# jiwoon-ahn/irn

Measured on NVIDIA H100. Metric: pseudo-label images/sec (CAM+random-walk), higher is better.
Workload: dtype f32

## Files before the change

### irn_b200/csrc/conv_wgmma.cuh

```cuda
#pragma once
#include <cuda.h>
#include <cuda_runtime.h>
#include <cstdint>
#include <type_traits>

#include "tma.cuh"

namespace irn {

constexpr int kTcTW = 16, kTcTH = 8;
constexpr int kTcBK = 32;
constexpr int kBfBK = 64;
constexpr int kWgThreads = 384;

struct TcMaps {
    CUtensorMap a;
    CUtensorMap b_hi;
    CUtensorMap b_lo;
    CUtensorMap a2;
};

struct TcArgs {
    const float* bias;
    const float* residual;
// ... 72 lines not shown
          "+f"(d[24]), "+f"(d[25]), "+f"(d[26]), "+f"(d[27]), "+f"(d[28]), "+f"(d[29]), "+f"(d[30]), "+f"(d[31]),
          "+f"(d[32]), "+f"(d[33]), "+f"(d[34]), "+f"(d[35]), "+f"(d[36]), "+f"(d[37]), "+f"(d[38]), "+f"(d[39]),
          "+f"(d[40]), "+f"(d[41]), "+f"(d[42]), "+f"(d[43]), "+f"(d[44]), "+f"(d[45]), "+f"(d[46]), "+f"(d[47]),
          "+f"(d[48]), "+f"(d[49]), "+f"(d[50]), "+f"(d[51]), "+f"(d[52]), "+f"(d[53]), "+f"(d[54]), "+f"(d[55]),
          "+f"(d[56]), "+f"(d[57]), "+f"(d[58]), "+f"(d[59]), "+f"(d[60]), "+f"(d[61]), "+f"(d[62]), "+f"(d[63])
        : "r"(a[0]), "r"(a[1]), "r"(a[2]), "r"(a[3]), "l"(db), "r"(scale_d));
}

template <> __device__ __forceinline__ void wg_mma<true, 64>(float (&d)[32], const uint32_t (&a)[4], uint64_t db, uint32_t scale_d) {
    asm volatile(
        "{\n\t.reg .pred p;\n\tsetp.ne.b32 p, %37, 0;\n\t"
        "wgmma.mma_async.sync.aligned.m64n64k16.f32.f16.f16 {"
        "%0, %1, %2, %3, %4, %5, %6, %7, %8, %9, %10, %11, %12, %13, %14, %15, "
        "%16, %17, %18, %19, %20, %21, %22, %23, %24, %25, %26, %27, %28, %29, %30, %31"
        "}, {%32, %33, %34, %35}, %36, p, 1, 1, 0;\n\t}"
        : "+f"(d[0]), "+f"(d[1]), "+f"(d[2]), "+f"(d[3]), "+f"(d[4]), "+f"(d[5]), "+f"(d[6]), "+f"(d[7]),
          "+f"(d[8]), "+f"(d[9]), "+f"(d[10]), "+f"(d[11]), "+f"(d[12]), "+f"(d[13]), "+f"(d[14]), "+f"(d[15]),
          "+f"(d[16]), "+f"(d[17]), "+f"(d[18]), "+f"(d[19]), "+f"(d[20]), "+f"(d[21]), "+f"(d[22]), "+f"(d[23]),
          "+f"(d[24]), "+f"(d[25]), "+f"(d[26]), "+f"(d[27]), "+f"(d[28]), "+f"(d[29]), "+f"(d[30]), "+f"(d[31])
        : "r"(a[0]), "r"(a[1]), "r"(a[2]), "r"(a[3]), "l"(db), "r"(scale_d));
}

template <> __device__ __forceinline__ void wg_mma<true, 128>(float (&d)[64], const uint32_t (&a)[4], uint64_t db, uint32_t scale_d) {
    asm volatile(
        "{\n\t.reg .pred p;\n\tsetp.ne.b32 p, %69, 0;\n\t"
        "wgmma.mma_async.sync.aligned.m64n128k16.f32.f16.f16 {"
        "%0, %1, %2, %3, %4, %5, %6, %7, %8, %9, %10, %11, %12, %13, %14, %15, "
        "%16, %17, %18, %19, %20, %21, %22, %23, %24, %25, %26, %27, %28, %29, %30, %31, "
        "%32, %33, %34, %35, %36, %37, %38, %39, %40, %41, %42, %43, %44, %45, %46, %47, "
        "%48, %49, %50, %51, %52, %53, %54, %55, %56, %57, %58, %59, %60, %61, %62, %63"
        "}, {%64, %65, %66, %67}, %68, p, 1, 1, 0;\n\t}"
        : "+f"(d[0]), "+f"(d[1]), "+f"(d[2]), "+f"(d[3]), "+f"(d[4]), "+f"(d[5]), "+f"(d[6]), "+f"(d[7]),
          "+f"(d[8]), "+f"(d[9]), "+f"(d[10]), "+f"(d[11]), "+f"(d[12]), "+f"(d[13]), "+f"(d[14]), "+f"(d[15]),
          "+f"(d[16]), "+f"(d[17]), "+f"(d[18]), "+f"(d[19]), "+f"(d[20]), "+f"(d[21]), "+f"(d[22]), "+f"(d[23]),
          "+f"(d[24]), "+f"(d[25]), "+f"(d[26]), "+f"(d[27]), "+f"(d[28]), "+f"(d[29]), "+f"(d[30]), "+f"(d[31]),
          "+f"(d[32]), "+f"(d[33]), "+f"(d[34]), "+f"(d[35]), "+f"(d[36]), "+f"(d[37]), "+f"(d[38]), "+f"(d[39]),
          "+f"(d[40]), "+f"(d[41]), "+f"(d[42]), "+f"(d[43]), "+f"(d[44]), "+f"(d[45]), "+f"(d[46]), "+f"(d[47]),
          "+f"(d[48]), "+f"(d[49]), "+f"(d[50]), "+f"(d[51]), "+f"(d[52]), "+f"(d[53]), "+f"(d[54]), "+f"(d[55]),
          "+f"(d[56]), "+f"(d[57]), "+f"(d[58]), "+f"(d[59]), "+f"(d[60]), "+f"(d[61]), "+f"(d[62]), "+f"(d[63])
        : "r"(a[0]), "r"(a[1]), "r"(a[2]), "r"(a[3]), "l"(db), "r"(scale_d));
}

__device__ __forceinline__ float tf32_hi(float x) { return __uint_as_float((__float_as_uint(x) + 0x1000u) & 0xFFFFE000u); }

__device__ __forceinline__ void f16_split2(float a, float b, uint32_t& hi, uint32_t& lo) {
    asm("cvt.rz.satfinite.f16x2.f32 %0, %1, %2;" : "=r"(hi) : "f"(b), "f"(a));
    const float ha = __uint_as_float(__float_as_uint(a) & 0xFFFFE000u), hb = __uint_as_float(__float_as_uint(b) & 0xFFFFE000u);
    asm("cvt.rn.satfinite.f16x2.f32 %0, %1, %2;" : "=r"(lo) : "f"(b - hb), "f"(a - ha));
}

template <bool F16>
__device__ __forceinline__ void wg_load_frag(const unsigned char* row, int k, int key, int t4, float (&v)[8]) {
    if (F16) {
        const unsigned char* box = row + (k >> 1) * 16384;
        const int c = 4 * (k & 1) + (t4 >> 1);
        const float2 x0 = *reinterpret_cast<const float2*>(box + ((c ^ key) << 4));
        const float2 x1 = *reinterpret_cast<const float2*>(box + 1024 + ((c ^ key) << 4));
        const float2 x2 = *reinterpret_cast<const float2*>(box + (((c + 2) ^ key) << 4));
        const float2 x3 = *reinterpret_cast<const float2*>(box + 1024 + (((c + 2) ^ key) << 4));
        v[0] = x0.x; v[1] = x0.y; v[2] = x1.x; v[3] = x1.y; v[4] = x2.x; v[5] = x2.y; v[6] = x3.x; v[7] = x3.y;
    } else {
        const int c = 2 * k;
        v[0] = *reinterpret_cast<const float*>(row + ((c ^ key) << 4));
        v[1] = *reinterpret_cast<const float*>(row + 1024 + ((c ^ key) << 4));
        v[2] = *reinterpret_cast<const float*>(row + (((c + 1) ^ key) << 4));
        v[3] = *reinterpret_cast<const float*>(row + 1024 + (((c + 1) ^ key) << 4));
    }
}

template <bool F16>
__device__ __forceinline__ void wg_split_frag(const float (&v)[8], uint32_t (&hi)[4], uint32_t (&lo)[4]) {
#pragma unroll
    for (int i = 0; i < 4; ++i) {
        if (F16) {
            f16_split2(v[2 * i], v[2 * i + 1], hi[i], lo[i]);
        } else {
            const float h = tf32_hi(v[i]);
            hi[i] = __float_as_uint(h);
            lo[i] = __float_as_uint(v[i] - h);
        }
    }
}

template <bool F16, int BN>
__global__ void __launch_bounds__(kWgThreads, 1)
conv_wg_kernel(const __grid_constant__ TcMaps maps, const TcArgs args) {
    using Cfg = WgCfg<F16, BN>;
    constexpr int S = Cfg::kStages;
    constexpr int R = BN / 2;
    extern __shared__ unsigned char wg_smem_raw[];
    unsigned char* smem = wg_smem_raw + ((1024u - (smem_u32(wg_smem_raw) & 1023u)) & 1023u);
    uint64_t* bars = (uint64_t*)(smem + S * Cfg::kStageBytes);
    uint64_t* full = bars;
    uint64_t* empty = bars + S;

    const int warp = threadIdx.x >> 5, lane = threadIdx.x & 31;
    const int n_tiles = args.Cout / BN;
    const int n_items = args.tiles_x * args.tiles_y * args.B * n_tiles;
    const int cblocks = args.Cin / Cfg::kBK;
    const int KB = (!F16 && args.stem) ? args.ksize : args.ksize * args.ksize * cblocks;

    if (threadIdx.x == 0) {
        for (int s = 0; s < S; ++s) {
            mbar_init(&full[s], 1);
            mbar_init(&empty[s], 8);
        }
        fence_mbar_init();
    }
    __syncthreads();

    if (warp < 4) {
        setmaxnreg_dec<kWgProducerRegs>();
        if (threadIdx.x == 0) {
            tma_prefetch_desc(&maps.a);
            tma_prefetch_desc(&maps.b_hi);
            tma_prefetch_desc(&maps.b_lo);
            if (F16 && args.kb_split < KB) tma_prefetch_desc(&maps.a2);
            int s = 0;
            uint32_t ph = 0;
            for (int item = blockIdx.x; item < n_items; item += gridDim.x) {
                const int tile = item / n_tiles;
                const int ox0 = (tile % args.tiles_x) * kTcTW;
                const int oy0 = ((tile / args.tiles_x) % args.tiles_y) * kTcTH;
                const int b = tile / (args.tiles_x * args.tiles_y);
                const int n0 = (item % n_tiles) * BN;
                for (int kb = 0; kb < KB; ++kb) {
                    mbar_wait(&empty[s], ph ^ 1);
                    unsigned char* st = smem + s * Cfg::kStageBytes;
                    unsigned char* wb = st + Cfg::kARaw;
                    mbar_arrive_expect_tx(&full[s], (uint32_t)Cfg::kStageBytes);
                    if (args.stem) {
                        const int row = F16 ? 2 * kb : kb;
                        tma_load_4d(st, &maps.a, &full[s], 0, ox0, oy0 * 2 + row, b);
                        if (F16) tma_load_4d(st + 16384, &maps.a, &full[s], 0, ox0, oy0 * 2 + row + 1, b);
                    } else {
                        const bool second = F16 && kb >= args.kb_split;
                        const CUtensorMap* am = second ? &maps.a2 : &maps.a;
                        const int tap = second ? 0 : kb / cblocks, cb = second ? kb - args.kb_split : kb % cblocks;
                        const int r = tap / args.ksize, ss = tap % args.ksize;
                        const int x = second ? ox0 * args.stride2 : ox0 * args.stride - args.pad + ss;
                        const int y = second ? oy0 * args.stride2 : oy0 * args.stride - args.pad + r;
                        tma_load_4d(st, am, &full[s], cb * Cfg::kBK, x, y, b);
                        if (F16) tma_load_4d(st + 16384, am, &full[s], cb * Cfg::kBK + 32, x, y, b);
                    }
                    tma_load_2d(wb, &maps.b_hi, &full[s], kb * Cfg::kBK, n0);
                    tma_load_2d(wb + Cfg::kBBytes, &maps.b_lo, &full[s], kb * Cfg::kBK, n0);
                    if (++s == S) { s = 0; ph ^= 1; }
                }
            }
        }
        return;
    }

    setmaxnreg_inc<kWgConsumerRegs>();
    const int g = (threadIdx.x >> 7) - 1, wq = warp & 3;
    const int key = lane >> 2, t4 = lane & 3;
    const int frag_off = (64 * g + 16 * wq + key) * 128 + (F16 ? 8 * (t4 & 1) : 4 * t4);
    float acc[R], part[2][R];
    uint32_t fa[2][2][4];
    int s = 0, s_prev = 0;
    uint32_t ph = 0;
    auto promote = [&](auto P) {
        constexpr int p = decltype(P)::value;
        wg_fence_regs(part[p]);
#pragma unroll
        for (int i = 0; i < R; ++i) acc[i] += part[p][i];
        __syncwarp();
        if (lane == 0) mbar_arrive(&empty[s_prev]);
    };
    auto kblock = [&](auto P) {
        constexpr int p = decltype(P)::value;
        mbar_wait(&full[s], ph);
        unsigned char* st = smem + s * Cfg::kStageBytes;
        const unsigned char* frag = st + frag_off;
        const uint32_t b_hi = smem_u32(st + Cfg::kARaw), b_lo = b_hi + Cfg::kBBytes;
#pragma unroll
        for (int k = 0; k < 4; ++k) {
            float v[8];
            wg_load_frag<F16>(frag, k, key, t4, v);
            wg_wait<1>();
            if (p == 1 && k == 1) promote(std::integral_constant<int, 0>());
            wg_split_frag<F16>(v, fa[k & 1][0], fa[k & 1][1]);
            if (k == 0) wg_fence_regs(part[p]);
            wg_fence();
            const uint64_t db_hi = wg_desc(b_hi + 32 * k), db_lo = wg_desc(b_lo + 32 * k);
            wg_mma<F16, BN>(part[p], fa[k & 1][0], db_hi, k != 0 ? 1u : 0u);
            wg_mma<F16, BN>(part[p], fa[k & 1][1], db_hi, 1u);
            wg_mma<F16, BN>(part[p], fa[k & 1][0], db_lo, 1u);
            wg_commit();
        }
        s_prev = s;
        if (++s == S) { s = 0; ph ^= 1; }
    };

    for (int item = blockIdx.x; item < n_items; item += gridDim.x) {
        const int tile = item / n_tiles;
        const int ox0 = (tile % args.tiles_x) * kTcTW;
        const int oy0 = ((tile / args.tiles_x) % args.tiles_y) * kTcTH;
        const int b = tile / (args.tiles_x * args.tiles_y);
        const int n0 = (item % n_tiles) * BN;
#pragma unroll
        for (int i = 0; i < R; ++i) acc[i] = 0.f;
        int kb = 0;
        for (; kb + 1 < KB; kb += 2) {
            kblock(std::integral_constant<int, 0>());
            kblock(std::integral_constant<int, 1>());
            wg_wait<0>();
            promote(std::integral_constant<int, 1>());
        }
        if (kb < KB) {
            kblock(std::integral_constant<int, 0>());
            wg_wait<0>();
            promote(std::integral_constant<int, 0>());
        }

#pragma unroll
        for (int h = 0; h < 2; ++h) {
            const int row = 64 * g + 16 * wq + (lane >> 2) + 8 * h;
            const int oy = oy0 + row / kTcTW, ox = ox0 + row % kTcTW;
            if (oy >= args.Ho || ox >= args.Wo) continue;
            const size_t base = (((size_t)b * args.Ho + oy) * args.Wo + ox) * args.Cout + n0 + 2 * (lane & 3);
#pragma unroll
            for (int j = 0; j < BN / 8; ++j) {
                const int n = n0 + 8 * j + 2 * (lane & 3);
                float2 o = make_float2(acc[4 * j + 2 * h], acc[4 * j + 2 * h + 1]);
                if (F16 && args.oscale) {
                    const float2 sc = __ldg(reinterpret_cast<const float2*>(args.oscale + n));
                    o.x *= sc.x; o.y *= sc.y;
                }
                if (args.bias) {
                    const float2 bi = __ldg(reinterpret_cast<const float2*>(args.bias + n));
                    o.x += bi.x; o.y += bi.y;
                }
                if (args.residual) {
                    const float2 rv = __ldg(reinterpret_cast<const float2*>(args.residual + base + 8 * j));
                    o.x += rv.x; o.y += rv.y;
                }
                if (args.relu) {
                    o.x = fmaxf(o.x, 0.f); o.y = fmaxf(o.y, 0.f);
                }
                *reinterpret_cast<float2*>(args.out + base + 8 * j) = o;
            }
        }
    }
}
#endif

}
```

### irn_b200/csrc/nets.cu

```cuda
#include <cuda_fp16.h>

#include <cmath>
#include <cstdlib>
#include <cstring>
#include <vector>

#include "common.h"
#include "conv_simt.cuh"
#include "conv_wgmma.cuh"

namespace irn {

struct Conv {
    int cin = 0, cout = 0, k = 1, stride = 1, pad = 0;
    float* wt = nullptr;
    float* bias = nullptr;
    float* w_hi = nullptr;
    float* w_lo = nullptr;
    int bn = 0;
    CUtensorMap map_bhi, map_blo;
    uint16_t* wb_hi = nullptr;
    uint16_t* wb_lo = nullptr;
    float* oscale = nullptr;
    bool bf_ok = false;
// ... 181 lines not shown
        IRN_CUDA(cudaMemcpy(host.data(), c.wt, host.size() * sizeof(float), cudaMemcpyDeviceToHost));
        const size_t K = 224;
        std::vector<float> hi(64 * K, 0.f), lo(64 * K, 0.f);
        for (int o = 0; o < 64; ++o)
            for (int r = 0; r < 7; ++r)
                for (int t = 0; t < 7; ++t)
                    for (int ci = 0; ci < 3; ++ci) {
                        const float v = host[((size_t)(r * 7 + t) * 3 + ci) * 64 + o];
                        uint32_t u;
                        std::memcpy(&u, &v, 4);
                        uint32_t h = (u + 0x1000u) & 0xFFFFE000u;
                        float hf;
                        std::memcpy(&hf, &h, 4);
                        if (!std::isfinite(hf)) hf = v;
                        hi[(size_t)o * K + r * 32 + t * 4 + ci] = hf;
                        lo[(size_t)o * K + r * 32 + t * 4 + ci] = v - hf;
                    }
        if ((rc = upload(net, hi, &c.w_hi))) return rc;
        if ((rc = upload(net, lo, &c.w_lo))) return rc;
        const uint64_t dims[2] = {K, 64};
        const uint64_t strides[1] = {K * sizeof(float)};
        const uint32_t box[2] = {(uint32_t)kTcBK, 64};
        if ((rc = make_tensor_map(&c.map_bhi, CU_TENSOR_MAP_DATA_TYPE_FLOAT32, 2, c.w_hi, dims, strides, box, CU_TENSOR_MAP_SWIZZLE_128B))) return rc;
        if ((rc = make_tensor_map(&c.map_blo, CU_TENSOR_MAP_DATA_TYPE_FLOAT32, 2, c.w_lo, dims, strides, box, CU_TENSOR_MAP_SWIZZLE_128B))) return rc;
        c.stem_tc = true;
        Conv& f = net->stem_f16;
        f.cin = 256; f.cout = 64; f.k = 1; f.stride = 1; f.pad = 0;
        std::vector<float> wt((size_t)256 * 64, 0.f);
        for (int o = 0; o < 64; ++o)
            for (int r = 0; r < 7; ++r)
                for (int t = 0; t < 7; ++t)
                    for (int ci = 0; ci < 3; ++ci)
                        wt[(size_t)(r * 32 + t * 4 + ci) * 64 + o] = host[((size_t)(r * 7 + t) * 3 + ci) * 64 + o];
        f.bias = c.bias;
        if ((rc = make_bf16_weights(net, f, wt))) return rc;
    }
    int cin = 64;
    for (int l = 0; l < 4; ++l) {
        net->blocks[l].resize(kBlocks[l]);
        for (int b = 0; b < kBlocks[l]; ++b) {
            Block& blk = net->blocks[l][b];
            const int planes = kPlanes[l], stride = b == 0 ? kStrides[l] : 1;
            if ((rc = read_conv(net, rd, blk.c1, cin, planes, 1, 1, 0, true))) return rc;
            if ((rc = read_conv(net, rd, blk.c2, planes, planes, 3, stride, 1, true))) return rc;
            if ((rc = read_conv(net, rd, blk.c3, planes, planes * 4, 1, 1, 0, true))) return rc;
            blk.has_ds = b == 0;
            if (blk.has_ds && (rc = read_conv(net, rd, blk.ds, cin, planes * 4, 1, stride, 0, true))) return rc;
            if (blk.has_ds && planes % kBfBK == 0 && cin % kBfBK == 0) {
                Conv& f = blk.c3ds;
                const int cout = planes * 4, K3 = planes, Kd = cin;
                f.cin = K3 + Kd; f.cout = cout; f.k = 1; f.stride = 1; f.pad = 0;
                std::vector<float> wt((size_t)(K3 + Kd) * cout), bias(cout);
                std::copy(blk.c3.host_wt.begin(), blk.c3.host_wt.end(), wt.begin());
                std::copy(blk.ds.host_wt.begin(), blk.ds.host_wt.end(), wt.begin() + (size_t)K3 * cout);
                for (int o = 0; o < cout; ++o) bias[o] = blk.c3.host_bias[o] + blk.ds.host_bias[o];
                if ((rc = upload(net, bias, &f.bias))) return rc;
                if ((rc = make_bf16_weights(net, f, wt))) return rc;
                blk.has_c3ds = f.bf_ok;
            }
            cin = planes * 4;
        }
    }
    net->stem.host_wt.clear(); net->stem.host_wt.shrink_to_fit();
    for (int l = 0; l < 4; ++l)
        for (Block& blk : net->blocks[l])
            for (Conv* c : {&blk.c1, &blk.c2, &blk.c3, &blk.ds}) {
                std::vector<float>().swap(c->host_wt);
                std::vector<float>().swap(c->host_bias);
            }
    return kOk;
}

static int read_head(irn_net* net, Reader& rd, Head& h, int cin, int cout, int groups, int up) {
    int rc = read_conv(net, rd, h.conv, cin, cout, 1, 1, 0, false);
    if (rc) return rc;
    h.groups = groups;
    h.up = up;
    if ((rc = read_vec(net, rd, cout, &h.gamma))) return rc;
    return read_vec(net, rd, cout, &h.beta);
}

static inline int conv_out(int n, int k, int s, int p) { return (n + 2 * p - k) / s + 1; }

template <bool F16, int BN>
static int launch_wg(const TcMaps& maps, const TcArgs& a, cudaStream_t st) {
    using Cfg = WgCfg<F16, BN>;
    static DeviceOnce once;
    const int ds = once.slot();
    if (once.need(ds)) {
        IRN_CUDA(cudaFuncSetAttribute((conv_wg_kernel<F16, BN>), cudaFuncAttributeMaxDynamicSharedMemorySize, (int)Cfg::kSmem));
        int dev = 0, n_sm = 0, per_sm = 0;
        IRN_CUDA(cudaGetDevice(&dev));
        IRN_CUDA(cudaDeviceGetAttribute(&n_sm, cudaDevAttrMultiProcessorCount, dev));
        IRN_CUDA(cudaOccupancyMaxActiveBlocksPerMultiprocessor(&per_sm, conv_wg_kernel<F16, BN>, kWgThreads, Cfg::kSmem));
        if (per_sm < 1) return fail(kCudaError, "conv_wg_kernel: no CTA fits on an SM (%zu bytes of shared memory)", Cfg::kSmem);
        once.n_sm[ds] = n_sm * per_sm;
        once.done[ds] = true;
    }
    const long long items = (long long)a.tiles_x * a.tiles_y * a.B * (a.Cout / BN);
    const long long grid = items < once.n_sm[ds] ? items : once.n_sm[ds];
    conv_wg_kernel<F16, BN><<<(unsigned)grid, kWgThreads, Cfg::kSmem, st>>>(maps, a);
    IRN_LAUNCH_CHECK(F16 ? "conv_wg_kernel<f16x3>" : "conv_wg_kernel<3xtf32>");
    return kOk;
}

static TcArgs conv_args(const Conv& c, int B, int Ho, int Wo, const float* residual, float* out, bool relu) {
    TcArgs a;
    a.bias = c.bias; a.residual = residual; a.out = out;
    a.oscale = c.oscale;
    a.B = B; a.Ho = Ho; a.Wo = Wo; a.Cout = c.cout; a.Cin = c.cin; a.ksize = c.k; a.stride = c.stride; a.pad = c.pad;
    a.relu = relu ? 1 : 0;
    a.tiles_x = (Wo + kTcTW - 1) / kTcTW;
    a.tiles_y = (Ho + kTcTH - 1) / kTcTH;
    return a;
}

static int act_map(CUtensorMap* m, const float* in, int B, int H, int W, int cin, int stride) {
    const uint64_t dims[4] = {(uint64_t)cin, (uint64_t)W, (uint64_t)H, (uint64_t)B};
    const uint64_t strides[3] = {(uint64_t)cin * 4, (uint64_t)W * cin * 4, (uint64_t)H * W * cin * 4};
    const uint32_t box[4] = {32u, (uint32_t)(kTcTW * stride), (uint32_t)(kTcTH * stride), 1};
    const uint32_t estr[4] = {1, (uint32_t)stride, (uint32_t)stride, 1};
    return make_tensor_map(m, CU_TENSOR_MAP_DATA_TYPE_FLOAT32, 4, in, dims, strides, box, CU_TENSOR_MAP_SWIZZLE_128B, estr);
}

static int stem_map(CUtensorMap* m, const float* x4, int B, int Hin, int Win) {
    const int Hp = Hin + 6, Wp = Win + 8;
    const int Wo = conv_out(Win, 7, 2, 3);
    const uint64_t dims[4] = {32, (uint64_t)Wo, (uint64_t)Hp, (uint64_t)B};
    const uint64_t strides[3] = {32, (uint64_t)Wp * 16, (uint64_t)Hp * Wp * 16};
    const uint32_t box[4] = {32, (uint32_t)kTcTW, (uint32_t)(kTcTH * 2), 1};
    const uint32_t estr[4] = {1, 1, 2, 1};
    return make_tensor_map(m, CU_TENSOR_MAP_DATA_TYPE_FLOAT32, 4, x4, dims, strides, box, CU_TENSOR_MAP_SWIZZLE_128B, estr);
}

static int run_conv_tf32(const Conv& c, const float* in, int B, int H, int W, int Ho, int Wo, const float* residual, float* out, bool relu,
                         cudaStream_t st) {
    TcMaps maps;
    maps.b_hi = c.map_bhi;
    maps.b_lo = c.map_blo;
    int rc = act_map(&maps.a, in, B, H, W, c.cin, c.stride);
    if (rc) return rc;
    maps.a2 = maps.a;
    TcArgs a = conv_args(c, B, Ho, Wo, residual, out, relu);
    a.oscale = nullptr;
    return c.bn == 128 ? launch_wg<false, 128>(maps, a, st) : launch_wg<false, 64>(maps, a, st);
}

static int launch_tf32_stem(const Conv& c, const float* x4, int B, int Hin, int Win, float* out, cudaStream_t st) {
    TcMaps maps;
    maps.b_hi = c.map_bhi;
    maps.b_lo = c.map_blo;
    int rc = stem_map(&maps.a, x4, B, Hin, Win);
    if (rc) return rc;
    maps.a2 = maps.a;
    TcArgs a = conv_args(c, B, conv_out(Hin, 7, 2, 3), conv_out(Win, 7, 2, 3), nullptr, out, true);
    a.oscale = nullptr;
    a.Cin = 32; a.ksize = 7; a.stride = 2; a.pad = 3; a.stem = 1;
    return launch_wg<false, 64>(maps, a, st);
}

struct F16Second {
    const float* in = nullptr;
    int H = 0, W = 0, cin = 0, stride = 1;
};

static int run_conv_f16(const Conv& c, const float* in, int B, int H, int W, int Ho, int Wo, const float* residual, float* out, bool relu,
                        cudaStream_t st, const F16Second* second = nullptr) {
    const bool wide = c.cout % 128 == 0;
    TcMaps maps;
    maps.b_hi = c.map_bf_hi[wide ? 1 : 0];
    maps.b_lo = c.map_bf_lo[wide ? 1 : 0];
    const int cin1 = second ? c.cin - second->cin : c.cin;
    int rc = act_map(&maps.a, in, B, H, W, cin1, c.stride);
    if (rc) return rc;
    maps.a2 = maps.a;
    TcArgs a = conv_args(c, B, Ho, Wo, residual, out, relu);
    if (second) {
        if (c.k != 1) return fail(kUnsupported, "run_conv_f16: a second input needs a 1x1 conv");
        if ((rc = act_map(&maps.a2, second->in, B, second->H, second->W, second->cin, second->stride))) return rc;
        a.kb_split = cin1 / kBfBK;
        a.stride2 = second->stride;
    }
    return wide ? launch_wg<true, 128>(maps, a, st) : launch_wg<true, 64>(maps, a, st);
}
// ... 381 lines not shown
```

### irn_b200/csrc/rw.cu

```cuda
#include <mutex>
#include <type_traits>

#include "common.h"
#include "path_tables.h"
#include "tma.cuh"

namespace irn {

constexpr int kMaxDst = 160;
constexpr int kMaxPts = 2304;

struct DevTables {
    int n_dst;
    int radius;
    short plane[kMaxDst];
    signed char dy[kMaxDst], dx[kMaxDst];
    short pstart[kMaxDst + 1];
    signed char py[kMaxPts], px[kMaxPts];
};
__constant__ DevTables c_tab;

static std::mutex g_tab_mutex;
static int g_tab_radius[64] = {0};
static int g_tab_ndst[64] = {0};
// ... 457 lines not shown
            static_for<0, 5>([&](auto CLS) {
                constexpr int cls = decltype(CLS)::value;
                const uint32_t slot = nw % NW;
                const float* wb = s_w + slot * kWBufFloats;
                mbar_wait(&fullW[slot], (nw / NW) & 1);
                ++nw;
                static_for<0, (cls == 0 ? 1 : 2)>([&](auto SGN) {
                    constexpr int dxc = decltype(SGN)::value == 0 ? cls : -cls;
                    static_for<-kR, kPY + kR>([&](auto RR) {
                        constexpr int r = decltype(RR)::value;
                        double v[CH];
#pragma unroll
                        for (int c = 0; c < CH; ++c) v[c] = sy[(c * kYH + ty0 + r + kR) * kSW + lane + dxc + kR];
                        static_for<0, kPY>([&](auto JJ) {
                            constexpr int j = decltype(JJ)::value;
                            constexpr int dy = r - j;
                            constexpr int kf = plane5(dy, dxc);
                            constexpr int kb = plane5(-dy, -dxc);
                            if constexpr (kf >= 0) {
                                const double wv = widen_weight(wb[((kf - cls_base5(cls)) * kWH + ty0 + j + kR) * kSW + lane + kR]);
#pragma unroll
                                for (int c = 0; c < CH; ++c) acc[j][c] = fma(wv, v[c], acc[j][c]);
                            } else if constexpr (kb >= 0) {
                                const double wv = widen_weight(wb[((kb - cls_base5(cls)) * kWH + ty0 + r + kR) * kSW + lane + dxc + kR]);
#pragma unroll
                                for (int c = 0; c < CH; ++c) acc[j][c] = fma(wv, v[c], acc[j][c]);
                            }
                        });
                    });
                });
                __syncwarp();
                if (lane == 0) mbar_arrive(&emptyW[slot]);
            });
            __syncwarp();
            if (lane == 0) mbar_arrive(&emptyY[ys]);

            if (x < w) {
#pragma unroll
                for (int j = 0; j < kPY; ++j) {
                    if (yb + j < h) {
                        const double is = inv_s[(size_t)img * plane_sz + (size_t)(yb + j) * pitch + x];
#pragma unroll
                        for (int c = 0; c < CH; ++c)
                            if (c0 + c < c_end) yout[(size_t)(c0 + c) * plane_sz + (size_t)(yb + j) * pitch + x] = acc[j][c] * is;
                    }
                }
            }
        }
    }
}
#endif

constexpr int kFR = 8;
constexpr int kFW = 128;
constexpr int kFYP = kFW + 2 * kR;
constexpr int kFYR = kFR + 2 * kR;
#ifndef IRN_RW_REGPLANES4
#define IRN_RW_REGPLANES4 16
#endif
#ifndef IRN_RW_REGPLANES2
#define IRN_RW_REGPLANES2 16
#endif
constexpr int fused_threads(int py) { return (kFW / 32) * (kFR / py) * 32; }

__host__ __device__ constexpr int plane_dy5(int k) {
    if (k < 4) return k + 1;
    for (int c = 1; c <= 4; ++c) {
        const int base = cls_base5(c), m = cls_maxdy5(c);
        if (k < base + m + 1) return k - base;
        if (k < base + 2 * m + 1) return k - base - m;
    }
    return 0;
}
__host__ __device__ constexpr int wrow_base5(int k) {
    int s = 0;
    for (int i = 0; i < k; ++i) s += kFR + plane_dy5(i);
    return s;
}
constexpr int kFWRows = wrow_base5(34);
static_assert(kFWRows == 340 && plane_dy5(plane5(3, -2)) == 3 && plane_dy5(plane5(0, 4)) == 0 && plane_dy5(plane5(4, 0)) == 4, "fused weight layout");
constexpr size_t kFusedWBytes = 16 + (size_t)kFWRows * kFW * sizeof(float) + 16;
constexpr size_t kFusedSmem = kFusedWBytes + 2 * (size_t)kFYR * kFYP * sizeof(double);

__device__ __forceinline__ uint32_t cluster_ctarank() {
    uint32_t r;
    asm volatile("mov.u32 %0, %%cluster_ctarank;" : "=r"(r));
    return r;
}
__device__ __forceinline__ uint32_t cluster_nctarank() {
    uint32_t r;
    asm volatile("mov.u32 %0, %%cluster_nctarank;" : "=r"(r));
    return r;
}
__device__ __forceinline__ void cluster_sync_all() {
    asm volatile("barrier.cluster.arrive.release.aligned;\n\tbarrier.cluster.wait.acquire.aligned;" ::: "memory");
}
__device__ __forceinline__ uint32_t cluster_map(uint32_t local_smem_addr, uint32_t rank) {
    uint32_t r;
    asm volatile("mapa.shared::cluster.u32 %0, %1, %2;" : "=r"(r) : "r"(local_smem_addr), "r"(rank));
    return r;
}
__device__ __forceinline__ void st_cluster_f64(uint32_t addr, double v) {
    asm volatile("st.shared::cluster.f64 [%0], %1;" ::"r"(addr), "d"(v) : "memory");
}

template <int kFPY>
__global__ void __launch_bounds__(fused_threads(kFPY), 1)
rw_fused_kernel(const float* __restrict__ W, const double* __restrict__ inv_s, const float* __restrict__ x,
                const float* __restrict__ edge, float* __restrict__ out, const int* __restrict__ chan_off, int totc, int h, int w,
                int pitch, int n_iter) {
    constexpr int kFThreads = fused_threads(kFPY);
    extern __shared__ __align__(128) unsigned char smem_raw[];
    float* s_w = (float*)(smem_raw + 16);
    double* s_y = (double*)(smem_raw + kFusedWBytes);

    const int tid = threadIdx.x, lane = tid & 31, warp = tid >> 5;
    const int rank = (int)cluster_ctarank(), csize = (int)cluster_nctarank();
    const int n_clusters = gridDim.x / csize, cid = blockIdx.x / csize;
    const int per = (totc + n_clusters - 1) / n_clusters;
    const int c_lo = cid * per, c_hi = c_lo + per < totc ? c_lo + per : totc;
    const int r0 = rank * kFR;
    const bool active = r0 < h;
    const int col = (warp & 3) * 32 + lane;
    const int ty0 = (warp >> 2) * kFPY;
    const size_t plane_sz = (size_t)h * pitch;
    const size_t hw = (size_t)h * w;

    if (tid < 4) {
        ((float*)smem_raw)[tid] = 0.f;
        ((float*)(smem_raw + kFusedWBytes - 16))[tid] = 0.f;
    }
    for (int i = tid; i < 2 * kFYR * kFYP; i += kFThreads) s_y[i] = 0.0;
    __syncthreads();
    cluster_sync_all();

    const uint32_t sy_addr = smem_u32(s_y);
    const uint32_t up_addr = rank > 0 ? cluster_map(sy_addr, (uint32_t)(rank - 1)) : 0u;
    const uint32_t dn_addr = rank + 1 < csize ? cluster_map(sy_addr, (uint32_t)(rank + 1)) : 0u;

    int cur_img = -1;
    constexpr int kRegPlanes = kFPY == 4 ? IRN_RW_REGPLANES4 : IRN_RW_REGPLANES2;
    float wf[kFPY][kRegPlanes > 0 ? kRegPlanes : 1];
    for (int c = c_lo; c < c_hi; ++c) {
        int img = 0;
        while (chan_off[img + 1] <= c) ++img;
        double val[kFPY], is[kFPY];
        if (active) {
            if (img != cur_img) {
                const float* Wi = W + (size_t)img * 34 * plane_sz;
                static_for<0, 34>([&](auto K) {
                    constexpr int k = decltype(K)::value;
                    constexpr int dyk = plane_dy5(k);
                    constexpr int rows = kFR + dyk;
                    float* dst = s_w + (size_t)wrow_base5(k) * kFW;
                    const float* src = Wi + (size_t)k * plane_sz;
                    for (int i = tid; i < rows * (kFW / 4); i += kFThreads) {
                        const int lr = i / (kFW / 4), c4 = (i % (kFW / 4)) * 4;
                        const int gr = r0 - dyk + lr;
                        float4 v = make_float4(0.f, 0.f, 0.f, 0.f);
                        if (gr >= 0 && gr < h && c4 < w) {
                            v = __ldg(reinterpret_cast<const float4*>(src + (size_t)gr * pitch + c4));
                            if (c4 + 1 >= w) v.y = 0.f;
                            if (c4 + 2 >= w) v.z = 0.f;
                            if (c4 + 3 >= w) v.w = 0.f;
                        }
                        *reinterpret_cast<float4*>(dst + lr * kFW + c4) = v;
                    }
                });
            }
            if (img != cur_img) {
                __syncthreads();
                static_for<0, kRegPlanes>([&](auto K) {
                    constexpr int k = decltype(K)::value;
#pragma unroll
                    for (int j = 0; j < kFPY; ++j) wf[j][k] = s_w[(wrow_base5(k) + plane_dy5(k) + ty0 + j) * kFW + col];
                });
            }
#pragma unroll
            for (int j = 0; j < kFPY; ++j) {
                const int gr = r0 + ty0 + j;
                const bool in = gr < h && col < w;
                is[j] = in ? inv_s[(size_t)img * plane_sz + (size_t)gr * pitch + col] : 0.0;
                val[j] = in ? (double)__fmul_rn(x[(size_t)c * hw + (size_t)gr * w + col], 1.0f - edge[(size_t)img * hw + (size_t)gr * w + col]) : 0.0;
            }
// ... 399 lines not shown
```

### irn_b200/csrc/tma.cuh

```cuda
#pragma once
#include <cuda.h>
#include <cuda_runtime.h>
#include <cstdint>

#include "common.h"

namespace irn {

typedef CUresult (*EncodeTiledFn)(CUtensorMap*, CUtensorMapDataType, cuuint32_t, void*, const cuuint64_t*,
                                  const cuuint64_t*, const cuuint32_t*, const cuuint32_t*, CUtensorMapInterleave,
                                  CUtensorMapSwizzle, CUtensorMapL2promotion, CUtensorMapFloatOOBfill);

inline EncodeTiledFn encode_tiled_fn() {
    static EncodeTiledFn fn = nullptr;
    if (!fn) {
        void* p = nullptr;
        cudaDriverEntryPointQueryResult q;
        if (cudaGetDriverEntryPoint("cuTensorMapEncodeTiled", &p, cudaEnableDefault, &q) == cudaSuccess &&
            q == cudaDriverEntryPointSuccess)
            fn = (EncodeTiledFn)p;
    }
    return fn;
}

// ... 4 lines not shown
    if (!fn) return fail(kCudaError, "cuTensorMapEncodeTiled entry point not available");
    cuuint64_t d[5], s[5];
    cuuint32_t b[5], e[5];
    for (int i = 0; i < rank; ++i) {
        d[i] = dims[i];
        b[i] = box[i];
        e[i] = elem_strides ? elem_strides[i] : 1;
        if (i + 1 < rank) s[i] = strides_bytes[i];
    }
    CUresult r = fn(map, dt, (cuuint32_t)rank, const_cast<void*>(base), d, s, b, e, CU_TENSOR_MAP_INTERLEAVE_NONE, swz,
                    CU_TENSOR_MAP_L2_PROMOTION_L2_128B, CU_TENSOR_MAP_FLOAT_OOB_FILL_NONE);
    if (r != CUDA_SUCCESS)
        return fail(kCudaError, "cuTensorMapEncodeTiled failed (CUresult %d; rank %d dims %llu,%llu,%llu box %u,%u,%u)", (int)r,
                    rank, (unsigned long long)dims[0], (unsigned long long)(rank > 1 ? dims[1] : 0),
                    (unsigned long long)(rank > 2 ? dims[2] : 0), box[0], rank > 1 ? box[1] : 0, rank > 2 ? box[2] : 0);
    return kOk;
}

#ifdef __CUDACC__
__device__ __forceinline__ uint32_t smem_u32(const void* p) { return (uint32_t)__cvta_generic_to_shared(p); }

__device__ __forceinline__ void mbar_init(uint64_t* bar, uint32_t count) {
    asm volatile("mbarrier.init.shared::cta.b64 [%0], %1;" ::"r"(smem_u32(bar)), "r"(count) : "memory");
}
__device__ __forceinline__ void fence_mbar_init() { asm volatile("fence.mbarrier_init.release.cluster;" ::: "memory"); }
__device__ __forceinline__ void fence_proxy_async() { asm volatile("fence.proxy.async.shared::cta;" ::: "memory"); }

__device__ __forceinline__ void mbar_arrive_expect_tx(uint64_t* bar, uint32_t bytes) {
    asm volatile("mbarrier.arrive.expect_tx.shared::cta.b64 _, [%0], %1;" ::"r"(smem_u32(bar)), "r"(bytes) : "memory");
}
__device__ __forceinline__ void mbar_arrive(uint64_t* bar) {
    asm volatile("mbarrier.arrive.shared::cta.b64 _, [%0];" ::"r"(smem_u32(bar)) : "memory");
}
__device__ __forceinline__ bool mbar_try_wait(uint64_t* bar, uint32_t parity) {
    uint32_t ok;
    asm volatile(
        "{\n\t.reg .pred p;\n\t"
        "mbarrier.try_wait.parity.shared::cta.b64 p, [%1], %2;\n\t"
        "selp.u32 %0, 1, 0, p;\n\t}"
        : "=r"(ok)
        : "r"(smem_u32(bar)), "r"(parity)
        : "memory");
    return ok != 0;
}
__device__ __forceinline__ void mbar_wait(uint64_t* bar, uint32_t parity) {
    for (uint32_t spin = 0; !mbar_try_wait(bar, parity); ++spin)
        if (spin > (1u << 26)) __trap();
}

__device__ __forceinline__ bool mbar_test_wait(uint64_t* bar, uint32_t parity) {
    uint32_t ok;
    asm volatile(
        "{\n\t.reg .pred p;\n\t"
        "mbarrier.test_wait.parity.shared::cta.b64 p, [%1], %2;\n\t"
        "selp.u32 %0, 1, 0, p;\n\t}"
        : "=r"(ok)
        : "r"(smem_u32(bar)), "r"(parity)
        : "memory");
    return ok != 0;
}
__device__ __forceinline__ void mbar_wait_spin(uint64_t* bar, uint32_t parity) {
    for (uint32_t spin = 0; !mbar_test_wait(bar, parity); ++spin)
        if (spin > (1u << 28)) __trap();
}

__device__ __forceinline__ void tma_load_3d(void* smem_dst, const CUtensorMap* map, uint64_t* bar, int c0, int c1, int c2) {
    asm volatile(
        "cp.async.bulk.tensor.3d.shared::cluster.global.mbarrier::complete_tx::bytes [%0], [%1, {%3, %4, %5}], [%2];"
        ::"r"(smem_u32(smem_dst)), "l"(map), "r"(smem_u32(bar)), "r"(c0), "r"(c1), "r"(c2)
        : "memory");
}
__device__ __forceinline__ void tma_load_4d(void* smem_dst, const CUtensorMap* map, uint64_t* bar, int c0, int c1, int c2, int c3) {
    asm volatile(
        "cp.async.bulk.tensor.4d.shared::cluster.global.mbarrier::complete_tx::bytes [%0], [%1, {%3, %4, %5, %6}], [%2];"
        ::"r"(smem_u32(smem_dst)), "l"(map), "r"(smem_u32(bar)), "r"(c0), "r"(c1), "r"(c2), "r"(c3)
        : "memory");
}
__device__ __forceinline__ void tma_load_2d(void* smem_dst, const CUtensorMap* map, uint64_t* bar, int c0, int c1) {
    asm volatile(
        "cp.async.bulk.tensor.2d.shared::cluster.global.mbarrier::complete_tx::bytes [%0], [%1, {%3, %4}], [%2];"
        ::"r"(smem_u32(smem_dst)), "l"(map), "r"(smem_u32(bar)), "r"(c0), "r"(c1)
        : "memory");
}
__device__ __forceinline__ void tma_prefetch_3d(const CUtensorMap* map, int c0, int c1, int c2) {
    asm volatile("cp.async.bulk.prefetch.tensor.3d.L2.global.tile [%0, {%1, %2, %3}];" ::"l"(map), "r"(c0), "r"(c1), "r"(c2) : "memory");
}
__device__ __forceinline__ void tma_prefetch_desc(const CUtensorMap* map) {
    asm volatile("prefetch.tensormap [%0];" ::"l"(map) : "memory");
}
#endif

}
```

Before: 91.59.

## Pair CTAs in 2-CTA clusters and multicast shared activation tiles via TMA

For f16x3 non-stem convolutions with an even number of output-channel tiles, the kernel now runs as 2-CTA clusters. The two CTAs work on adjacent channel tiles of the same spatial tile. Each CTA loads one of the two 32-channel activation boxes and multicasts it to both CTAs, halving per-CTA activation loads from L2. Stage-release barriers now count arrivals from both CTAs' consumers, and a drain loop keeps a CTA from exiting while its peer still writes into it. The cost is that the paired CTAs run in lockstep and the grid is capped by the number of active clusters.

```diff
diff --git a/irn_b200/csrc/conv_wgmma.cuh b/irn_b200/csrc/conv_wgmma.cuh
--- a/irn_b200/csrc/conv_wgmma.cuh
+++ b/irn_b200/csrc/conv_wgmma.cuh
@@ -178,9 +178,10 @@
     }
 }
 
-template <bool F16, int BN>
+template <bool F16, int BN, bool PAIR>
 __global__ void __launch_bounds__(kWgThreads, 1)
 conv_wg_kernel(const __grid_constant__ TcMaps maps, const TcArgs args) {
+    static_assert(F16 || !PAIR, "pairs share the two 32-channel boxes of an f16x3 activation k-block");
     using Cfg = WgCfg<F16, BN>;
     constexpr int S = Cfg::kStages;
     constexpr int R = BN / 2;
@@ -199,11 +200,12 @@
     if (threadIdx.x == 0) {
         for (int s = 0; s < S; ++s) {
             mbar_init(&full[s], 1);
-            mbar_init(&empty[s], 8);
+            mbar_init(&empty[s], PAIR ? 16 : 8);
         }
         fence_mbar_init();
     }
-    __syncthreads();
+    if (PAIR) cluster_sync_all();
+    else __syncthreads();
 
     if (warp < 4) {
         setmaxnreg_dec<kWgProducerRegs>();
@@ -236,13 +238,22 @@
                         const int r = tap / args.ksize, ss = tap % args.ksize;
                         const int x = second ? ox0 * args.stride2 : ox0 * args.stride - args.pad + ss;
                         const int y = second ? oy0 * args.stride2 : oy0 * args.stride - args.pad + r;
-                        tma_load_4d(st, am, &full[s], cb * Cfg::kBK, x, y, b);
-                        if (F16) tma_load_4d(st + 16384, am, &full[s], cb * Cfg::kBK + 32, x, y, b);
+                        if (PAIR) {
+                            const int rank = (int)cluster_ctarank();
+                            tma_load_4d_mc(st + 16384 * rank, am, &full[s], 3, cb * Cfg::kBK + 32 * rank, x, y, b);
+                        } else {
+                            tma_load_4d(st, am, &full[s], cb * Cfg::kBK, x, y, b);
+                            if (F16) tma_load_4d(st + 16384, am, &full[s], cb * Cfg::kBK + 32, x, y, b);
+                        }
                     }
                     tma_load_2d(wb, &maps.b_hi, &full[s], kb * Cfg::kBK, n0);
                     tma_load_2d(wb + Cfg::kBBytes, &maps.b_lo, &full[s], kb * Cfg::kBK, n0);
                     if (++s == S) { s = 0; ph ^= 1; }
                 }
+            }
+            for (int i = 0; PAIR && i < S; ++i) {
+                mbar_wait(&empty[s], ph ^ 1);
+                if (++s == S) { s = 0; ph ^= 1; }
             }
         }
         return;
@@ -262,7 +273,14 @@
 #pragma unroll
         for (int i = 0; i < R; ++i) acc[i] += part[p][i];
         __syncwarp();
-        if (lane == 0) mbar_arrive(&empty[s_prev]);
+        if (lane == 0) {
+            if (PAIR) {
+                mbar_arrive_cluster(&empty[s_prev], 0);
+                mbar_arrive_cluster(&empty[s_prev], 1);
+            } else {
+                mbar_arrive(&empty[s_prev]);
+            }
+        }
     };
     auto kblock = [&](auto P) {
         constexpr int p = decltype(P)::value;
diff --git a/irn_b200/csrc/nets.cu b/irn_b200/csrc/nets.cu
--- a/irn_b200/csrc/nets.cu
+++ b/irn_b200/csrc/nets.cu
@@ -287,24 +287,59 @@
 
 static inline int conv_out(int n, int k, int s, int p) { return (n + 2 * p - k) / s + 1; }
 
+template <int BN>
+static int launch_wg_pair(const TcMaps& maps, const TcArgs& a, cudaStream_t st) {
+    using Cfg = WgCfg<true, BN>;
+    static DeviceOnce once;
+    cudaLaunchConfig_t cfg = {};
+    cfg.gridDim = dim3(2);
+    cfg.blockDim = dim3(kWgThreads);
+    cfg.dynamicSmemBytes = Cfg::kSmem;
+    cfg.stream = st;
+    cudaLaunchAttribute attr[1];
+    attr[0].id = cudaLaunchAttributeClusterDimension;
+    attr[0].val.clusterDim.x = 2;
+    attr[0].val.clusterDim.y = 1;
+    attr[0].val.clusterDim.z = 1;
+    cfg.attrs = attr;
+    cfg.numAttrs = 1;
+    const int ds = once.slot();
+    if (once.need(ds)) {
+        IRN_CUDA(cudaFuncSetAttribute((conv_wg_kernel<true, BN, true>), cudaFuncAttributeMaxDynamicSharedMemorySize, (int)Cfg::kSmem));
+        int clusters = 0;
+        IRN_CUDA(cudaOccupancyMaxActiveClusters(&clusters, conv_wg_kernel<true, BN, true>, &cfg));
+        if (clusters < 1) return fail(kCudaError, "conv_wg_kernel: no 2-CTA cluster fits (%zu bytes of shared memory per CTA)", Cfg::kSmem);
+        once.n_sm[ds] = clusters;
+        once.done[ds] = true;
+    }
+    const long long pairs = (long long)a.tiles_x * a.tiles_y * a.B * (a.Cout / BN) / 2;
+    cfg.gridDim = dim3((unsigned)(2 * (pairs < once.n_sm[ds] ? pairs : once.n_sm[ds])));
+    IRN_CUDA(cudaLaunchKernelEx(&cfg, conv_wg_kernel<true, BN, true>, maps, a));
+    IRN_LAUNCH_CHECK("conv_wg_kernel<f16x3, pair>");
+    return kOk;
+}
+
 template <bool F16, int BN>
 static int launch_wg(const TcMaps& maps, const TcArgs& a, cudaStream_t st) {
+    if constexpr (F16) {
+        if ((a.Cout / BN) % 2 == 0 && !a.stem) return launch_wg_pair<BN>(maps, a, st);
+    }
     using Cfg = WgCfg<F16, BN>;
     static DeviceOnce once;
     const int ds = once.slot();
     if (once.need(ds)) {
-        IRN_CUDA(cudaFuncSetAttribute((conv_wg_kernel<F16, BN>), cudaFuncAttributeMaxDynamicSharedMemorySize, (int)Cfg::kSmem));
+        IRN_CUDA(cudaFuncSetAttribute((conv_wg_kernel<F16, BN, false>), cudaFuncAttributeMaxDynamicSharedMemorySize, (int)Cfg::kSmem));
         int dev = 0, n_sm = 0, per_sm = 0;
         IRN_CUDA(cudaGetDevice(&dev));
         IRN_CUDA(cudaDeviceGetAttribute(&n_sm, cudaDevAttrMultiProcessorCount, dev));
-        IRN_CUDA(cudaOccupancyMaxActiveBlocksPerMultiprocessor(&per_sm, conv_wg_kernel<F16, BN>, kWgThreads, Cfg::kSmem));
+        IRN_CUDA(cudaOccupancyMaxActiveBlocksPerMultiprocessor(&per_sm, conv_wg_kernel<F16, BN, false>, kWgThreads, Cfg::kSmem));
         if (per_sm < 1) return fail(kCudaError, "conv_wg_kernel: no CTA fits on an SM (%zu bytes of shared memory)", Cfg::kSmem);
         once.n_sm[ds] = n_sm * per_sm;
         once.done[ds] = true;
     }
     const long long items = (long long)a.tiles_x * a.tiles_y * a.B * (a.Cout / BN);
     const long long grid = items < once.n_sm[ds] ? items : once.n_sm[ds];
-    conv_wg_kernel<F16, BN><<<(unsigned)grid, kWgThreads, Cfg::kSmem, st>>>(maps, a);
+    conv_wg_kernel<F16, BN, false><<<(unsigned)grid, kWgThreads, Cfg::kSmem, st>>>(maps, a);
     IRN_LAUNCH_CHECK(F16 ? "conv_wg_kernel<f16x3>" : "conv_wg_kernel<3xtf32>");
     return kOk;
 }
diff --git a/irn_b200/csrc/rw.cu b/irn_b200/csrc/rw.cu
--- a/irn_b200/csrc/rw.cu
+++ b/irn_b200/csrc/rw.cu
@@ -563,24 +563,6 @@
 constexpr size_t kFusedWBytes = 16 + (size_t)kFWRows * kFW * sizeof(float) + 16;
 constexpr size_t kFusedSmem = kFusedWBytes + 2 * (size_t)kFYR * kFYP * sizeof(double);
 
-__device__ __forceinline__ uint32_t cluster_ctarank() {
-    uint32_t r;
-    asm volatile("mov.u32 %0, %%cluster_ctarank;" : "=r"(r));
-    return r;
-}
-__device__ __forceinline__ uint32_t cluster_nctarank() {
-    uint32_t r;
-    asm volatile("mov.u32 %0, %%cluster_nctarank;" : "=r"(r));
-    return r;
-}
-__device__ __forceinline__ void cluster_sync_all() {
-    asm volatile("barrier.cluster.arrive.release.aligned;\n\tbarrier.cluster.wait.acquire.aligned;" ::: "memory");
-}
-__device__ __forceinline__ uint32_t cluster_map(uint32_t local_smem_addr, uint32_t rank) {
-    uint32_t r;
-    asm volatile("mapa.shared::cluster.u32 %0, %1, %2;" : "=r"(r) : "r"(local_smem_addr), "r"(rank));
-    return r;
-}
 __device__ __forceinline__ void st_cluster_f64(uint32_t addr, double v) {
     asm volatile("st.shared::cluster.f64 [%0], %1;" ::"r"(addr), "d"(v) : "memory");
 }
diff --git a/irn_b200/csrc/tma.cuh b/irn_b200/csrc/tma.cuh
--- a/irn_b200/csrc/tma.cuh
+++ b/irn_b200/csrc/tma.cuh
@@ -110,6 +110,36 @@
         ::"r"(smem_u32(smem_dst)), "l"(map), "r"(smem_u32(bar)), "r"(c0), "r"(c1)
         : "memory");
 }
+__device__ __forceinline__ void tma_load_4d_mc(void* smem_dst, const CUtensorMap* map, uint64_t* bar, uint16_t mask, int c0, int c1,
+                                               int c2, int c3) {
+    asm volatile(
+        "cp.async.bulk.tensor.4d.shared::cluster.global.mbarrier::complete_tx::bytes.multicast::cluster [%0], [%1, {%4, %5, %6, %7}], [%2], %3;"
+        ::"r"(smem_u32(smem_dst)), "l"(map), "r"(smem_u32(bar)), "h"(mask), "r"(c0), "r"(c1), "r"(c2), "r"(c3)
+        : "memory");
+}
+
+__device__ __forceinline__ uint32_t cluster_ctarank() {
+    uint32_t r;
+    asm volatile("mov.u32 %0, %%cluster_ctarank;" : "=r"(r));
+    return r;
+}
+__device__ __forceinline__ uint32_t cluster_nctarank() {
+    uint32_t r;
+    asm volatile("mov.u32 %0, %%cluster_nctarank;" : "=r"(r));
+    return r;
+}
+__device__ __forceinline__ void cluster_sync_all() {
+    asm volatile("barrier.cluster.arrive.release.aligned;\n\tbarrier.cluster.wait.acquire.aligned;" ::: "memory");
+}
+__device__ __forceinline__ uint32_t cluster_map(uint32_t local_smem_addr, uint32_t rank) {
+    uint32_t r;
+    asm volatile("mapa.shared::cluster.u32 %0, %1, %2;" : "=r"(r) : "r"(local_smem_addr), "r"(rank));
+    return r;
+}
+__device__ __forceinline__ void mbar_arrive_cluster(uint64_t* bar, uint32_t rank) {
+    asm volatile("mbarrier.arrive.shared::cluster.b64 _, [%0];" ::"r"(cluster_map(smem_u32(bar), rank)) : "memory");
+}
+
 __device__ __forceinline__ void tma_prefetch_3d(const CUtensorMap* map, int c0, int c1, int c2) {
     asm volatile("cp.async.bulk.prefetch.tensor.3d.L2.global.tile [%0, {%1, %2, %3}];" ::"l"(map), "r"(c0), "r"(c1), "r"(c2) : "memory");
 }
```

Result: no change. 92.36, median of 6 (+0.8%).
